# facebookresearch/multipathnet

Hardware: NVIDIA H100
Metric: proposals/sec (higher is better)
Workload: dtype fp32 (wgmma split emulation, fp32 accumulate: 3 bf16 products per MAC, 2 fp16 products in fc6/fc7)

## Files before the change

### multipathnet_b200/csrc/gemm_tc.cu

```cuda
#include "conv_gemm.cuh"
#include "wgmma.cuh"
#include "fp8_e4m3.cuh"
#include <algorithm>
#include <stdlib.h>
#include <string.h>

namespace {

constexpr int BM = 128;
constexpr int BK = 64;
constexpr int TC_THREADS = 384;
constexpr int CONS_THREADS = 256;
constexpr int A_TILE_BYTES = BM * BK * 2;
constexpr int SMEM_BUDGET = 196608;

__host__ __device__ constexpr int a_planes(OperandScheme ops) { return (ops == OperandScheme::BF16X1 || ops == OperandScheme::FP8X1) ? 1 : 2; }
__host__ __device__ constexpr int b_planes(OperandScheme ops) { return ops == OperandScheme::BF16X3 ? 2 : 1; }
__host__ __device__ constexpr int elem_bytes(OperandScheme ops) { return ops == OperandScheme::FP8X1 ? 1 : 2; }
__host__ __device__ constexpr int row_bytes(int BN, OperandScheme ops) { return (ops == OperandScheme::FP8X1 || BN == 256) ? 64 : 128; }
__host__ __device__ constexpr int stage_k(int BN, OperandScheme ops) { return row_bytes(BN, ops) / elem_bytes(ops); }
__host__ __device__ constexpr int kb_steps(int BN, OperandScheme ops) { return BK / stage_k(BN, ops); }
__host__ __device__ constexpr int a_tile_bytes(int BN, OperandScheme ops) { return BM * row_bytes(BN, ops); }
__host__ __device__ constexpr int stage_bytes(int BN, OperandScheme ops = OperandScheme::BF16X3) {
  return (a_planes(ops) * BM + b_planes(ops) * BN) * row_bytes(BN, ops);
}
__host__ __device__ constexpr int max_stages(int BN, OperandScheme ops) { return row_bytes(BN, ops) == 64 ? 8 : 4; }
__host__ __device__ constexpr int num_stages(int BN, OperandScheme ops = OperandScheme::BF16X3) {
  return (SMEM_BUDGET / stage_bytes(BN, ops)) > max_stages(BN, ops) ? max_stages(BN, ops) : (SMEM_BUDGET / stage_bytes(BN, ops));
}
constexpr int EPI_WARP_BYTES = 16 * 128;
constexpr int EPI_BYTES = (CONS_THREADS / 32) * EPI_WARP_BYTES;
__host__ __device__ constexpr int tc_smem_bytes(int BN, OperandScheme ops) {
  return num_stages(BN, ops) * stage_bytes(BN, ops) + EPI_BYTES + 1024  + 256 ;
}

struct TcParams {
  int N, Ho, Wo, Cout;
  int kh, kw, stride, pad;
  int cblocks;
  int tn, th, tw;
  int tiles_img, tiles_h, tiles_w, tiles_n;
  int units;
  const float *bias;
  const __nv_bfloat16 *res_hi, *res_lo; long long res_ld;
  __nv_bfloat16 *out_hi, *out_lo; long long out_ld;
  float *out_f32; long long out_f32_ld;
  __nv_bfloat16 *pool_hi, *pool_lo; long long pool_ld; int Hp, Wp;
  int relu;
  int splitk, kb_per_split;
  long long split_stride;
  unsigned long long *tl_min, *tl_max;
  float acc_scale;
  int out_fmt;
  unsigned *ovf;
  const int *a_exp, *b_exp; long long sample_pix;
};

__device__ __forceinline__ unsigned long long gtimer() {
  unsigned long long t; asm volatile("mov.u64 %0, %%globaltimer;" : "=l"(t)); return t;
}
__device__ __forceinline__ void tl_min_stamp(const unsigned long long *base_, int i) {
  if (base_) atomicMin(const_cast<unsigned long long *>(base_) + i, gtimer());
}
__device__ __forceinline__ void tl_max_stamp(const unsigned long long *base_, int i) {
  if (base_) atomicMax(const_cast<unsigned long long *>(base_) + i, gtimer());
}
__device__ __forceinline__ uint32_t smem_u32(const void *p) { return (uint32_t)__cvta_generic_to_shared(p); }
__device__ __forceinline__ void mbar_init(uint32_t bar, uint32_t count) {
  asm volatile("mbarrier.init.shared::cta.b64 [%0], %1;" ::"r"(bar), "r"(count) : "memory");
}
__device__ __forceinline__ void mbar_expect_tx(uint32_t bar, uint32_t bytes) {
  asm volatile("mbarrier.arrive.expect_tx.shared::cta.b64 _, [%0], %1;" ::"r"(bar), "r"(bytes) : "memory");
}
__device__ __forceinline__ void mbar_arrive(uint32_t bar) {
  asm volatile("mbarrier.arrive.shared::cta.b64 _, [%0];" ::"r"(bar) : "memory");
}
__device__ __forceinline__ void mbar_wait(uint32_t bar, uint32_t parity) {
  uint32_t done;
  uint32_t spins = 0;
  do {
    asm volatile(
        "{\n\t.reg .pred p;\n\t"
        "mbarrier.try_wait.parity.shared::cta.b64 p, [%1], %2;\n\t"
        "selp.u32 %0, 1, 0, p;\n\t}"
        : "=r"(done) : "r"(bar), "r"(parity) : "memory");
    if (!done && ++spins == (1u << 26)) __trap();
  } while (!done);
}
__device__ __forceinline__ void tma_load_4d(uint32_t dst, const CUtensorMap *tm, uint32_t bar, int c0, int c1,
                                            int c2, int c3) {
  asm volatile(
      "cp.async.bulk.tensor.4d.shared::cluster.global.mbarrier::complete_tx::bytes [%0], [%1, {%3, %4, %5, %6}], [%2];"
      ::"r"(dst), "l"(reinterpret_cast<uint64_t>(tm)), "r"(bar), "r"(c0), "r"(c1), "r"(c2), "r"(c3) : "memory");
}
__device__ __forceinline__ void tma_load_2d(uint32_t dst, const CUtensorMap *tm, uint32_t bar, int c0, int c1) {
  asm volatile(
      "cp.async.bulk.tensor.2d.shared::cluster.global.mbarrier::complete_tx::bytes [%0], [%1, {%3, %4}], [%2];"
      ::"r"(dst), "l"(reinterpret_cast<uint64_t>(tm)), "r"(bar), "r"(c0), "r"(c1) : "memory");
}
__device__ __forceinline__ void prefetch_tmap(const CUtensorMap *tm) {
  asm volatile("prefetch.tensormap [%0];" ::"l"(reinterpret_cast<uint64_t>(tm)) : "memory");
}

__device__ __forceinline__ uint64_t make_smem_desc(uint32_t saddr) {
  uint64_t d = 0;
  d |= (uint64_t)((saddr & 0x3FFFFu) >> 4);
  d |= (uint64_t)1 << 16;
  d |= (uint64_t)(1024 >> 4) << 32;
  d |= (uint64_t)1 << 62;
  return d;
}

__device__ __forceinline__ uint64_t make_smem_desc_64b(uint32_t saddr) {
  uint64_t d = 0;
  d |= (uint64_t)((saddr & 0x3FFFFu) >> 4);
  d |= (uint64_t)1 << 16;
  d |= (uint64_t)(512 >> 4) << 32;
  d |= (uint64_t)2 << 62;
  return d;
}

template <int BN, OperandScheme OPS>
__device__ __forceinline__ void mma_kstep(float (&acc)[BN / 2], uint64_t a_hi, uint64_t a_lo, uint64_t b_hi, uint64_t b_lo, bool first) {
  constexpr bool F16 = (OPS == OperandScheme::FP16X2);
#pragma unroll
  for (int k = 0; k < stage_k(BN, OPS) / 16; ++k) {
    const uint64_t adv = (uint64_t)((k * 16 * 2) >> 4);
    const uint32_t later = (first && k == 0) ? 0u : 1u;
    if constexpr (OPS == OperandScheme::BF16X1) {
      wgmma_nk16<BN, false>(acc, a_hi + adv, b_hi + adv, later);
    } else {
      wgmma_nk16<BN, F16>(acc, a_lo + adv, b_hi + adv, later);
      if (!F16) wgmma_nk16<BN, F16>(acc, a_hi + adv, b_lo + adv, 1u);
      wgmma_nk16<BN, F16>(acc, a_hi + adv, b_hi + adv, 1u);
    }
  }
}

struct UnitPos { int nt, twi, thi, tni, split; };
__device__ __forceinline__ UnitPos unit_pos(const TcParams &p, int unit) {
  UnitPos u;
  const int tile = unit / p.splitk;
  u.split = unit - tile * p.splitk;
  u.nt = tile % p.tiles_n;
  const int mt = tile / p.tiles_n;
  u.twi = mt % p.tiles_w; u.thi = (mt / p.tiles_w) % p.tiles_h; u.tni = mt / (p.tiles_w * p.tiles_h);
  return u;
}
__device__ __forceinline__ long long row_pixel(const TcParams &p, const UnitPos &u, int row, bool &ok, int *whn = nullptr) {
  const int lw = __ffs(p.tw) - 1, lh = __ffs(p.th) - 1;
  const int wl = row & (p.tw - 1), hl = (row >> lw) & (p.th - 1), nl = row >> (lw + lh);
  const int wo = u.twi * p.tw + wl, ho = u.thi * p.th + hl, n = u.tni * p.tn + nl;
  ok = (wo < p.Wo) && (ho < p.Ho) && (n < p.N);
  if (whn) { whn[0] = wo; whn[1] = ho; whn[2] = n; }
  return ((long long)n * p.Ho + ho) * p.Wo + wo;
}

__device__ __forceinline__ void store_plane_chunk(uint32_t so, const uint32_t (&v)[16], __nv_bfloat16 *out, long long ld,
                                                  const TcParams &p, const UnitPos &u, int rbase, int col0, int lane) {
  const int r = lane >> 2;
  const uint32_t wr = so + (uint32_t)(r * 128 + 4 * (lane & 3));
  __syncwarp();
#pragma unroll
  for (int j = 0; j < 8; ++j) {
    const uint32_t a = wr + (uint32_t)((j ^ r) * 16);
    asm volatile("st.shared.b32 [%0], %1;" ::"r"(a), "r"(v[j]) : "memory");
    asm volatile("st.shared.b32 [%0], %1;" ::"r"(a + 8 * 128), "r"(v[8 + j]) : "memory");
  }
  __syncwarp();
  const int row0 = lane >> 3, ch = lane & 7;
  const uint32_t rd0 = so + (uint32_t)(row0 * 128 + ((ch ^ row0) * 16)), rd1 = so + (uint32_t)(row0 * 128 + ((ch ^ row0 ^ 4) * 16));
  const bool col_ok = col0 + 8 * ch < p.Cout;
#pragma unroll
  for (int q = 0; q < 4; ++q) {
    uint4 d;
    asm volatile("ld.shared.v4.b32 {%0, %1, %2, %3}, [%4];" : "=r"(d.x), "=r"(d.y), "=r"(d.z), "=r"(d.w)
                 : "r"(((q & 1) ? rd1 : rd0) + (uint32_t)(q * 4 * 128)) : "memory");
    bool ok;
    const long long pix = row_pixel(p, u, rbase + 4 * q + row0, ok);
    if (ok && col_ok) *reinterpret_cast<uint4 *>(out + pix * ld + col0 + 8 * ch) = d;
  }
}

template <int BN, OperandScheme OPS>
__device__ __forceinline__ void tile_epilogue(const TcParams &p, const UnitPos &u, float (&acc)[BN / 2], int g, int wq,
                                              int lane, uint32_t so) {
  const int rbase = 64 * g + 16 * wq;
  const int c0 = 2 * (lane & 3);
  bool fok[2]; long long fpix[2];
#pragma unroll
  for (int i = 0; i < 2; ++i) fpix[i] = row_pixel(p, u, rbase + (lane >> 2) + 8 * i, fok[i]);
  int ea[2] = {0, 0};
  if constexpr (OPS == OperandScheme::FP8X1) {
#pragma unroll
    for (int i = 0; i < 2; ++i) ea[i] = fok[i] ? __ldg(p.a_exp + fpix[i] / p.sample_pix) : 0;
  }
  const bool pool = (p.pool_hi != nullptr);
  bool pok = false; long long ppix = 0;
  if (pool) {
    int whn[3];
    row_pixel(p, u, rbase + 2 * (lane >> 3), pok, whn);
    ppix = ((long long)whn[2] * p.Hp + (whn[1] >> 1)) * p.Wp + (whn[0] >> 1);
  }
  float *const out_f32 = p.out_f32 ? p.out_f32 + (long long)u.split * p.split_stride : nullptr;
#pragma unroll 1
  for (int m = 0; m < BN / 64; ++m) {
    const int col0 = u.nt * BN + 64 * m;
    if (col0 >= p.Cout) break;
    float *f = acc;
#pragma unroll
    for (int j = 0; j < 8; ++j) {
      const int c = col0 + 8 * j + c0;
      const bool full8 = col0 + 8 * j + 8 <= p.Cout;
      float b[2] = {0.f, 0.f};
      int eb[2] = {0, 0};
#pragma unroll
      for (int k = 0; k < 2; ++k) {
        if (p.bias && c + k < p.Cout) b[k] = __ldg(p.bias + c + k);
        if constexpr (OPS == OperandScheme::FP8X1) eb[k] = __ldg(p.b_exp + c + k);
      }
#pragma unroll
      for (int i = 0; i < 2; ++i) {
        float &f0 = f[4 * j + 2 * i], &f1 = f[4 * j + 2 * i + 1];
        if constexpr (OPS == OperandScheme::FP16X2) { f0 *= p.acc_scale; f1 *= p.acc_scale; }
        if constexpr (OPS == OperandScheme::FP8X1) {
          f0 *= mpn_fp8::pow2(-(ea[i] + eb[0])); f1 *= mpn_fp8::pow2(-(ea[i] + eb[1]));
        }
        if (p.bias) {
          if (c < p.Cout) f0 += b[0];
          if (c + 1 < p.Cout) f1 += b[1];
        }
        if (p.res_hi && full8 && fok[i]) {
          const float2 x = bf16x2_to_float2(*reinterpret_cast<const uint32_t *>(p.res_hi + fpix[i] * p.res_ld + c));
          const float2 y = bf16x2_to_float2(*reinterpret_cast<const uint32_t *>(p.res_lo + fpix[i] * p.res_ld + c));
          f0 += x.x + y.x; f1 += x.y + y.y;
        }
        if (p.relu) { f0 = fmaxf(f0, 0.f); f1 = fmaxf(f1, 0.f); }
        if (out_f32 && fok[i]) {
          float *o = out_f32 + fpix[i] * p.out_f32_ld + c;
          if (c < p.Cout) o[0] = f0;
          if (c + 1 < p.Cout) o[1] = f1;
        }
      }
    }
    float mx[16];
    if (pool) {
#pragma unroll
      for (int j = 0; j < 8; ++j)
#pragma unroll
        for (int k = 0; k < 2; ++k) {
          float top = fok[0] ? f[4 * j + k] : -INFINITY, bot = fok[1] ? f[4 * j + 2 + k] : -INFINITY;
          top = fmaxf(top, __shfl_xor_sync(0xffffffffu, top, 4));
          bot = fmaxf(bot, __shfl_xor_sync(0xffffffffu, bot, 4));
          mx[2 * j + k] = fmaxf(top, bot);
        }
    }
#pragma unroll 1
    for (int plane = 0; plane < 2; ++plane) {
      if (p.out_hi) {
        uint32_t v[16];
#pragma unroll
        for (int j = 0; j < 8; ++j)
#pragma unroll
          for (int i = 0; i < 2; ++i) {
            uint32_t hi2 = 0, lo2 = 0;
            if (fok[i]) split_x2(p.out_fmt, f[4 * j + 2 * i], f[4 * j + 2 * i + 1], hi2, lo2, p.ovf);
            v[8 * i + j] = plane ? lo2 : hi2;
          }
        store_plane_chunk(so, v, plane ? p.out_lo : p.out_hi, p.out_ld, p, u, rbase, col0, lane);
      }
      if (pool) {
        const int pr = lane >> 3;
        __syncwarp();
        if (!(lane & 4) && fok[0]) {
#pragma unroll
          for (int j = 0; j < 8; ++j) {
            uint32_t hi2, lo2;
            split_x2(p.out_fmt, mx[2 * j], mx[2 * j + 1], hi2, lo2, p.ovf);
            const uint32_t a = so + (uint32_t)(pr * 128 + ((j ^ pr) * 16) + 4 * (lane & 3));
            asm volatile("st.shared.b32 [%0], %1;" ::"r"(a), "r"(plane ? lo2 : hi2) : "memory");
          }
        }
        __syncwarp();
        const int ch = lane & 7;
        uint4 d;
        asm volatile("ld.shared.v4.b32 {%0, %1, %2, %3}, [%4];" : "=r"(d.x), "=r"(d.y), "=r"(d.z), "=r"(d.w)
                     : "r"(so + (uint32_t)(pr * 128 + ((ch ^ pr) * 16))) : "memory");
        if (pok && col0 + 8 * ch < p.Cout)
          *reinterpret_cast<uint4 *>((plane ? p.pool_lo : p.pool_hi) + ppix * p.pool_ld + col0 + 8 * ch) = d;
      }
    }
#pragma unroll
    for (int k = 0; k + 32 < BN / 2; ++k) acc[k] = acc[k + 32];
  }
}

template <int BN, OperandScheme OPS = OperandScheme::BF16X3>
__global__ void __launch_bounds__(TC_THREADS, 1)
conv_gemm_tc_kernel(const __grid_constant__ CUtensorMap tmA_hi, const __grid_constant__ CUtensorMap tmA_lo,
                    const __grid_constant__ CUtensorMap tmB_hi, const __grid_constant__ CUtensorMap tmB_lo,
                    const TcParams p) {
  constexpr int S = num_stages(BN, OPS);
  constexpr int STAGE = stage_bytes(BN, OPS);
  constexpr int A_TILE = a_tile_bytes(BN, OPS);
  constexpr int B_TILE_BYTES = BN * row_bytes(BN, OPS);
  constexpr int B_OFF = a_planes(OPS) * A_TILE;
  constexpr int KSTEPS = kb_steps(BN, OPS);
  static_assert(S >= 2 && 2 * S * 8 <= 256, "ring depth: at least two stages, barriers in their 256 bytes");
  extern __shared__ uint8_t smem_raw[];
  uint8_t *smem = reinterpret_cast<uint8_t *>((reinterpret_cast<uintptr_t>(smem_raw) + 1023) & ~(uintptr_t)1023);
  uint64_t *bars = reinterpret_cast<uint64_t *>(smem + (size_t)S * STAGE + EPI_BYTES);
  const uint32_t smem_base = smem_u32(smem);
  const uint32_t bar_base = smem_u32(bars);
  auto full_bar = [&](int s) { return bar_base + 8u * s; };
  auto empty_bar = [&](int s) { return bar_base + 8u * (S + s); };

  const int tid = threadIdx.x, lane = tid & 31;
  const int num_kb = p.kh * p.kw * p.cblocks;

  if (tid == 0) {
    tl_min_stamp(p.tl_min, 0);
    if (a_planes(OPS) == 1) { prefetch_tmap(&tmA_hi); prefetch_tmap(&tmB_hi); }
    else { prefetch_tmap(&tmA_hi); prefetch_tmap(&tmA_lo); prefetch_tmap(&tmB_hi); prefetch_tmap(&tmB_lo); }
    for (int s = 0; s < S; ++s) { mbar_init(full_bar(s), 1); mbar_init(empty_bar(s), CONS_THREADS / 32); }
    asm volatile("fence.mbarrier_init.release.cluster;" ::: "memory");
  }
  __syncthreads();
  asm volatile("griddepcontrol.wait;" ::: "memory");
  asm volatile("griddepcontrol.launch_dependents;" ::: "memory");
  if (tid == 0) tl_min_stamp(p.tl_min, 1);

  if (tid < 128) {
    asm volatile("setmaxnreg.dec.sync.aligned.u32 24;" ::: "memory");
    if (tid == 0) {
      int it = 0;
      for (int unit = (int)blockIdx.x; unit < p.units; unit += (int)gridDim.x) {
        const UnitPos u = unit_pos(p, unit);
        const int kb0 = u.split * p.kb_per_split, kb1 = min(num_kb, kb0 + p.kb_per_split);
        const int w_in0 = u.twi * p.tw * p.stride - p.pad, h_in0 = u.thi * p.th * p.stride - p.pad, n0 = u.tni * p.tn;
        const int b_row0 = u.nt * BN;
        for (int kb = kb0; kb < kb1; ++kb) {
          const int tap = kb / p.cblocks, cb = kb - tap * p.cblocks;
          const int khi = tap / p.kw, kwi = tap - khi * p.kw;
#pragma unroll
          for (int h = 0; h < KSTEPS; ++h, ++it) {
            const int s = it % S; const uint32_t ph = (uint32_t)(it / S) & 1u;
            const int ka = cb * BK + h * stage_k(BN, OPS), kk = kb * BK + h * stage_k(BN, OPS);
            mbar_wait(empty_bar(s), ph ^ 1u);
            const uint32_t sa = smem_base + (uint32_t)s * STAGE;
            mbar_expect_tx(full_bar(s), (uint32_t)STAGE);
            tma_load_4d(sa, &tmA_hi, full_bar(s), ka, w_in0 + kwi, h_in0 + khi, n0);
            if (a_planes(OPS) == 2) tma_load_4d(sa + A_TILE, &tmA_lo, full_bar(s), ka, w_in0 + kwi, h_in0 + khi, n0);
            tma_load_2d(sa + B_OFF, &tmB_hi, full_bar(s), kk, b_row0);
            if (b_planes(OPS) == 2) tma_load_2d(sa + B_OFF + B_TILE_BYTES, &tmB_lo, full_bar(s), kk, b_row0);
          }
        }
      }
    }
    return;
  }

  asm volatile("setmaxnreg.inc.sync.aligned.u32 240;" ::: "memory");
  const int e = tid - 128;
  const int g = e >> 7, wq = (e >> 5) & 3;
  const uint32_t so = smem_base + (uint32_t)(S * STAGE + (e >> 5) * EPI_WARP_BYTES);
  int it = 0;
  for (int unit = (int)blockIdx.x; unit < p.units; unit += (int)gridDim.x) {
    const UnitPos u = unit_pos(p, unit);
    const int kb0 = u.split * p.kb_per_split, kb1 = min(num_kb, kb0 + p.kb_per_split);
    float acc[BN / 2];
#pragma unroll
    for (int i = 0; i < BN / 2; ++i) acc[i] = 0.f;
    if constexpr (OPS == OperandScheme::FP8X1) {
      float part[BN / 2];
#pragma unroll
      for (int i = 0; i < BN / 2; ++i) part[i] = 0.f;
      for (int kb = kb0; kb < kb1; ++kb, ++it) {
        const int s = it % S; const uint32_t ph = (uint32_t)(it / S) & 1u;
        mbar_wait(full_bar(s), ph);
        if (it == 0 && e == 0) tl_min_stamp(p.tl_min, 2);
        const uint32_t sa = smem_base + (uint32_t)s * STAGE;
        const uint64_t a8 = make_smem_desc_64b(sa + (uint32_t)g * (A_TILE / 2));
        const uint64_t b8 = make_smem_desc_64b(sa + B_OFF);
#pragma unroll
        for (int k = 0; k < BK / 32; ++k) {
          wgmma_fence_acc(part);
          wgmma_fence();
          wgmma_e4m3_nk32<BN>(part, a8 + (uint64_t)(2 * k), b8 + (uint64_t)(2 * k), 0u);
          wgmma_commit();
          wgmma_wait<0>();
          wgmma_fence_acc(part);
#pragma unroll
          for (int i = 0; i < BN / 2; ++i) acc[i] += part[i];
        }
        if (lane == 0) mbar_arrive(empty_bar(s));
      }
    } else {
      const int steps = (kb1 - kb0) * KSTEPS;
      for (int i = 0; i < steps; ++i, ++it) {
        const int s = it % S; const uint32_t ph = (uint32_t)(it / S) & 1u;
        mbar_wait(full_bar(s), ph);
        if (it == 0 && e == 0) tl_min_stamp(p.tl_min, 2);
        const uint32_t sa = smem_base + (uint32_t)s * STAGE;
        auto desc = [](uint32_t a) { return row_bytes(BN, OPS) == 64 ? make_smem_desc_64b(a) : make_smem_desc(a); };
        const uint64_t a_hi = desc(sa + (uint32_t)g * (A_TILE / 2));
        const uint64_t a_lo = desc(sa + A_TILE + (uint32_t)g * (A_TILE / 2));
        const uint64_t b_hi = desc(sa + B_OFF);
        const uint64_t b_lo = desc(sa + B_OFF + B_TILE_BYTES);
        wgmma_fence_acc(acc);
        wgmma_fence();
        mma_kstep<BN, OPS>(acc, a_hi, a_lo, b_hi, b_lo, i == 0);
        wgmma_commit();
        wgmma_wait<1>();
        wgmma_fence_acc(acc);
        if (i > 0 && lane == 0) mbar_arrive(empty_bar((it - 1) % S));
      }
      wgmma_wait<0>();
      wgmma_fence_acc(acc);
      if (lane == 0) mbar_arrive(empty_bar((it - 1) % S));
    }
    if (e == 0) tl_max_stamp(p.tl_max, 0);
    const uint32_t t_epi = (p.tl_max && e == 0) ? (uint32_t)gtimer() : 0u;
    tile_epilogue<BN, OPS>(p, u, acc, g, wq, lane, so);
    if (e == 0) {
      tl_max_stamp(p.tl_max, 1);
      if (p.tl_max) atomicAdd(p.tl_max + 3, (unsigned long long)((uint32_t)gtimer() - t_epi));
    }
  }
}


constexpr int C1_THREADS = 256;
constexpr int C1_A_BYTES = 2 * A_TILE_BYTES;
constexpr int C1_B_BYTES = 2 * 64 * 128;
constexpr int C1_OUT_WARP = 16 * 128;
constexpr int C1_SMEM = 2 * C1_A_BYTES + C1_B_BYTES + (C1_THREADS / 32) * C1_OUT_WARP + 1024;

__device__ __forceinline__ void conv1_gather(const float *__restrict__ x, int pix, int pixels, int H, int W, int bhalf,
                                             float (&in)[16]) {
#pragma unroll
  for (int k = 0; k < 16; ++k) in[k] = 0.f;
  if (pix < pixels) {
    const int HW = H * W;
    const int n = pix / HW, rem = pix - n * HW;
    const int ho = rem / W, wo = rem - ho * W;
    const float *x0 = x + ((size_t)n * 3 * HW + (size_t)(ho - 1) * W + (wo - 1));
    const bool rok[3] = {ho >= 1, true, ho + 1 < H}, cok[3] = {wo >= 1, true, wo + 1 < W};
#pragma unroll
    for (int k = 0; k < 16; ++k) {
      const int kk = 16 * bhalf + k;
      if (kk < 27) {
        const int ci = kk / 9, r = (kk / 3) % 3, q = kk % 3;
        in[k] = (rok[r] && cok[q]) ? __ldg(x0 + ci * HW + r * W + q) : 0.f;
      }
    }
  }
}

__device__ __forceinline__ void conv1_store_plane(uint32_t so, const uint32_t (&v)[16], __nv_bfloat16 *out, int pix0,
                                                  int pixels, int lane) {
  const int r = lane >> 2;
  const uint32_t wr = so + (uint32_t)(r * 128 + 4 * (lane & 3));
  __syncwarp();
#pragma unroll
  for (int j = 0; j < 8; ++j) {
    const uint32_t a = wr + (uint32_t)((j ^ r) * 16);
    asm volatile("st.shared.b32 [%0], %1;" ::"r"(a), "r"(v[j]) : "memory");
    asm volatile("st.shared.b32 [%0], %1;" ::"r"(a + 8 * 128), "r"(v[8 + j]) : "memory");
  }
  __syncwarp();
  const int row0 = lane >> 3, ch = lane & 7;
  const uint32_t rd0 = so + (uint32_t)(row0 * 128 + ((ch ^ row0) * 16)), rd1 = so + (uint32_t)(row0 * 128 + ((ch ^ row0 ^ 4) * 16));
  __nv_bfloat16 *o = out + (size_t)(pix0 + row0) * 64 + ch * 8;
#pragma unroll
  for (int q = 0; q < 4; ++q) {
    uint4 d;
    asm volatile("ld.shared.v4.b32 {%0, %1, %2, %3}, [%4];" : "=r"(d.x), "=r"(d.y), "=r"(d.z), "=r"(d.w)
                 : "r"(((q & 1) ? rd1 : rd0) + (uint32_t)(q * 4 * 128)) : "memory");
    if (pix0 + row0 + 4 * q < pixels) *reinterpret_cast<uint4 *>(o + q * 4 * 64) = d;
  }
}

__global__ void __launch_bounds__(C1_THREADS, 2)
conv1_tc_kernel(const float *__restrict__ x, int N, int H, int W, const float *__restrict__ w, const float *__restrict__ bias,
                int relu, __nv_bfloat16 *__restrict__ out_hi, __nv_bfloat16 *__restrict__ out_lo) {
  extern __shared__ uint8_t smem_raw[];
  uint8_t *smem = reinterpret_cast<uint8_t *>((reinterpret_cast<uintptr_t>(smem_raw) + 1023) & ~(uintptr_t)1023);
  uint8_t *sB = smem + 2 * C1_A_BYTES;
  const int tid = threadIdx.x, lane = tid & 31, warp = tid >> 5;
  const uint32_t so = smem_u32(sB + C1_B_BYTES) + (uint32_t)(warp * C1_OUT_WARP);
  const uint32_t b_base = smem_u32(sB);
  const int g = tid >> 7;
  const int pixels = N * H * W;
  const int total_tiles = (pixels + BM - 1) / BM;
  asm volatile("griddepcontrol.wait;" ::: "memory");
  asm volatile("griddepcontrol.launch_dependents;" ::: "memory");
  const int c0 = 2 * (lane & 3);
  for (int i = tid; i < 64 * 4; i += C1_THREADS) {
    const int row = i >> 2, j = i & 3;
    uint32_t hh[4], ll[4];
#pragma unroll
    for (int q = 0; q < 4; ++q) {
      const int k0 = j * 8 + 2 * q;
      const float v0 = (k0 < 27) ? __ldg(w + row * 27 + k0) : 0.f, v1 = (k0 + 1 < 27) ? __ldg(w + row * 27 + k0 + 1) : 0.f;
      split_bf16x2(v0, v1, hh[q], ll[q]);
    }
    const uint32_t off = (uint32_t)row * 128u + (uint32_t)((j ^ (row & 7)) * 16);
    *reinterpret_cast<uint4 *>(sB + off) = make_uint4(hh[0], hh[1], hh[2], hh[3]);
    *reinterpret_cast<uint4 *>(sB + 64 * 128 + off) = make_uint4(ll[0], ll[1], ll[2], ll[3]);
  }
  const int brow = tid & 127, bhalf = tid >> 7;
  float in[16];
  conv1_gather(x, (int)blockIdx.x * BM + brow, pixels, H, W, bhalf, in);
  for (int tile = blockIdx.x, it = 0; tile < total_tiles; tile += gridDim.x, ++it) {
    uint8_t *sa = smem + (it & 1) * C1_A_BYTES;
    uint8_t *pa = sa + (size_t)brow * 128;
#pragma unroll
    for (int jj = 0; jj < 2; ++jj) {
      const int j = 2 * bhalf + jj;
      uint32_t hh[4], ll[4];
#pragma unroll
      for (int q = 0; q < 4; ++q) split_bf16x2(in[jj * 8 + 2 * q], in[jj * 8 + 2 * q + 1], hh[q], ll[q]);
      const int pj = (j ^ (brow & 7)) * 16;
      *reinterpret_cast<uint4 *>(pa + pj) = make_uint4(hh[0], hh[1], hh[2], hh[3]);
      *reinterpret_cast<uint4 *>(pa + A_TILE_BYTES + pj) = make_uint4(ll[0], ll[1], ll[2], ll[3]);
    }
    asm volatile("fence.proxy.async.shared::cta;" ::: "memory");
    __syncthreads();
    float acc[32];
#pragma unroll
    for (int i = 0; i < 32; ++i) acc[i] = 0.f;
    const uint32_t a_base = smem_u32(sa);
    const uint64_t a_hi = make_smem_desc(a_base + (uint32_t)g * (A_TILE_BYTES / 2));
    const uint64_t a_lo = make_smem_desc(a_base + A_TILE_BYTES + (uint32_t)g * (A_TILE_BYTES / 2));
    const uint64_t b_hi = make_smem_desc(b_base), b_lo = make_smem_desc(b_base + 64 * 128);
    wgmma_fence_acc(acc);
    wgmma_fence();
#pragma unroll
    for (int k = 0; k < 2; ++k) {
      const uint64_t adv = (uint64_t)((k * 16 * 2) >> 4);
      wgmma_nk16<64, false>(acc, a_lo + adv, b_hi + adv, k ? 1u : 0u);
      wgmma_nk16<64, false>(acc, a_hi + adv, b_lo + adv, 1u);
      wgmma_nk16<64, false>(acc, a_hi + adv, b_hi + adv, 1u);
    }
    wgmma_commit();
    const int next = tile + (int)gridDim.x;
    conv1_gather(x, next < total_tiles ? next * BM + brow : pixels, pixels, H, W, bhalf, in);
    wgmma_wait<0>();
    wgmma_fence_acc(acc);
#pragma unroll
    for (int j = 0; j < 8; ++j) {
      const float2 b = __ldg(reinterpret_cast<const float2 *>(bias + 8 * j + c0));
#pragma unroll
      for (int h = 0; h < 2; ++h) {
        float &f0 = acc[4 * j + 2 * h], &f1 = acc[4 * j + 2 * h + 1];
        f0 += b.x; f1 += b.y;
        if (relu) { f0 = fmaxf(f0, 0.f); f1 = fmaxf(f1, 0.f); }
      }
    }
    const int pix0 = tile * BM + 64 * g + 16 * (warp & 3);
#pragma unroll 1
    for (int plane = 0; plane < 2; ++plane) {
      uint32_t v[16];
#pragma unroll
      for (int j = 0; j < 8; ++j)
#pragma unroll
        for (int h = 0; h < 2; ++h) {
          uint32_t hi2, lo2;
          split_bf16x2(acc[4 * j + 2 * h], acc[4 * j + 2 * h + 1], hi2, lo2);
          v[8 * h + j] = plane ? lo2 : hi2;
        }
      conv1_store_plane(so, v, plane ? out_lo : out_hi, pix0, pixels, lane);
    }
  }
}

struct ReduceParams {
  const float *ws; long long split_stride; int splitk; long long pixels; int Cout;
  const float *bias; const __nv_bfloat16 *res_hi, *res_lo; long long res_ld; int relu;
  __nv_bfloat16 *out_hi, *out_lo; long long out_ld; float *out_f32; long long out_f32_ld;
  OutScatter scatter;
};
__global__ void __launch_bounds__(256) splitk_reduce_kernel(const ReduceParams r) {
  MPN_PDL_SYNC();
  const long long idx = (long long)blockIdx.x * blockDim.x + threadIdx.x;
  if (idx >= r.pixels * r.Cout) return;
  const long long pix = idx / r.Cout; const int c = (int)(idx - pix * r.Cout);
  float acc = 0.f;
  for (int s = 0; s < r.splitk; ++s) acc += r.ws[(long long)s * r.split_stride + idx];
  if (r.bias) acc += __ldg(r.bias + c);
  if (r.res_hi) acc += join_bf16(r.res_hi[pix * r.res_ld + c], r.res_lo[pix * r.res_ld + c]);
  if (r.relu) acc = fmaxf(acc, 0.f);
  if (r.out_hi) { __nv_bfloat16 h, l; split_bf16(acc, h, l); r.out_hi[pix * r.out_ld + c] = h; r.out_lo[pix * r.out_ld + c] = l; }
  if (r.scatter.n > 0) {
#pragma unroll 1
    for (int g = 0; g < r.scatter.n; ++g)
      if (c >= r.scatter.seg[g].c0 && c < r.scatter.seg[g].c1) { r.scatter.seg[g].ptr[pix * r.scatter.seg[g].ld + (c - r.scatter.seg[g].c0)] = acc; break; }
  } else if (r.out_f32) r.out_f32[pix * r.out_f32_ld + c] = acc;
}

typedef CUresult (*PFN_encodeTiled)(CUtensorMap *, CUtensorMapDataType, cuuint32_t, void *, const cuuint64_t *,
                                    const cuuint64_t *, const cuuint32_t *, const cuuint32_t *, CUtensorMapInterleave,
                                    CUtensorMapSwizzle, CUtensorMapL2promotion, CUtensorMapFloatOOBfill);
PFN_encodeTiled get_encode_fn() {
  static PFN_encodeTiled fn = nullptr;
  if (!fn) {
    void *p = nullptr; cudaDriverEntryPointQueryResult q;
    if (cudaGetDriverEntryPoint("cuTensorMapEncodeTiled", &p, cudaEnableDefault, &q) == cudaSuccess &&
        q == cudaDriverEntryPointSuccess)
      fn = reinterpret_cast<PFN_encodeTiled>(p);
  }
  return fn;
}

int encode_map(mpn_ctx *ctx, CUtensorMap *tm, const void *base, int rank, const cuuint64_t *dims,
               const cuuint64_t *strides_bytes , const cuuint32_t *box, const cuuint32_t *estr, int BN, OperandScheme ops) {
  const bool fp8 = ops == OperandScheme::FP8X1;
  PFN_encodeTiled fn = get_encode_fn();
  if (!fn) return mpn_fail(ctx, MPN_ERR_CUDA, "cuTensorMapEncodeTiled entry point unavailable");
  CUresult r = fn(tm, fp8 ? CU_TENSOR_MAP_DATA_TYPE_UINT8 : CU_TENSOR_MAP_DATA_TYPE_BFLOAT16, (cuuint32_t)rank, const_cast<void *>(base), dims,
                  strides_bytes, box, estr, CU_TENSOR_MAP_INTERLEAVE_NONE, row_bytes(BN, ops) == 64 ? CU_TENSOR_MAP_SWIZZLE_64B : CU_TENSOR_MAP_SWIZZLE_128B,
                  CU_TENSOR_MAP_L2_PROMOTION_L2_256B, CU_TENSOR_MAP_FLOAT_OOB_FILL_NONE);
  if (r != CUDA_SUCCESS) {
    char b[256];
    snprintf(b, sizeof b, "cuTensorMapEncodeTiled failed (%d): rank %d dims %llu %llu box %u %u", (int)r, rank,
             (unsigned long long)dims[0], (unsigned long long)dims[1], box[0], box[1]);
    return mpn_fail(ctx, MPN_ERR_CUDA, b);
  }
  return MPN_OK;
}

inline bool tc_use_pdl() {
  static const int on = [] { const char *e = getenv("MPN_TC_PDL"); return (e && e[0] == '0') ? 0 : 1; }();
  return on != 0;
}

template <int BN, OperandScheme OPS = OperandScheme::BF16X3>
int launch_bn(mpn_ctx *ctx, const ConvPlan &pl, const TcParams &tp) {
  const int smem = tc_smem_bytes(BN, OPS);
  constexpr int bslot = BN == 256 ? 2 : (BN == 128 ? 1 : 0);
  constexpr int slot = OPS == OperandScheme::FP16X2 ? 3 : (OPS == OperandScheme::BF16X1 ? 5 + bslot
                                                         : (OPS == OperandScheme::FP8X1 ? 8 + bslot : bslot));
  if (!ctx->tc_attr_set[slot]) {
    MPN_CUDA(ctx, cudaFuncSetAttribute(conv_gemm_tc_kernel<BN, OPS>, cudaFuncAttributeMaxDynamicSharedMemorySize, smem));
    ctx->tc_attr_set[slot] = 1;
  }
  const long long units = (long long)pl.tiles_img * pl.tiles_h * pl.tiles_w * pl.tiles_n * pl.splitk;
  MPN_CHECK_ARG(ctx, units > 0 && units < (1ll << 31), "conv_tc: grid size out of range");
  TcParams tpu = tp;
  tpu.units = (int)units;
  cudaLaunchConfig_t cfg = {};
  cfg.gridDim = dim3((unsigned)std::min<long long>(units, ctx->sm_count));
  cfg.blockDim = dim3(TC_THREADS); cfg.dynamicSmemBytes = (size_t)smem; cfg.stream = ctx->stream;
  cudaLaunchAttribute attr[1];
  int na = 0;
  if (tc_use_pdl()) {
    attr[na].id = cudaLaunchAttributeProgrammaticStreamSerialization;
    attr[na].val.programmaticStreamSerializationAllowed = 1;
    ++na;
  }
  cfg.attrs = attr; cfg.numAttrs = na;
  MPN_CUDA(ctx, cudaLaunchKernelEx(&cfg, conv_gemm_tc_kernel<BN, OPS>, pl.tmA_hi, pl.tmA_lo, pl.tmB_hi, pl.tmB_lo, tpu));
  MPN_LAUNCHED(ctx);
  return MPN_OK;
}

int launch_ops(mpn_ctx *ctx, const ConvPlan &pl, const TcParams &tp) {
  if (pl.ops == OperandScheme::FP16X2) return launch_bn<256, OperandScheme::FP16X2>(ctx, pl, tp);
  if (pl.ops == OperandScheme::FP8X1)
    return pl.BN == 128 ? launch_bn<128, OperandScheme::FP8X1>(ctx, pl, tp) : launch_bn<64, OperandScheme::FP8X1>(ctx, pl, tp);
  if (pl.ops == OperandScheme::BF16X1) {
    switch (pl.BN) {
      case 256: return launch_bn<256, OperandScheme::BF16X1>(ctx, pl, tp);
      case 128: return launch_bn<128, OperandScheme::BF16X1>(ctx, pl, tp);
      default: return launch_bn<64, OperandScheme::BF16X1>(ctx, pl, tp);
    }
  }
  switch (pl.BN) {
    case 256: return launch_bn<256>(ctx, pl, tp);
    case 128: return launch_bn<128>(ctx, pl, tp);
    default: return launch_bn<64>(ctx, pl, tp);
  }
}

}

int conv1_tc_launch(mpn_ctx *ctx, const float *x_nchw, int N, int H, int W, const float *w_dev, const float *bias_dev, int relu,
                    DTensor &y) {
  MPN_CHECK_ARG(ctx, y.hi && y.lo && y.C == 64 && y.ld % 8 == 0, "conv1_tc: output must be 64-channel split planes");
  MPN_CHECK_ARG(ctx, bias_dev, "conv1_tc: bias missing");
  MPN_CHECK_ARG(ctx, y.ld == 64 && (long long)N * H * W < (1ll << 31) - 256, "conv1_tc: dense 64-channel output and < 2^31 pixels");
  if (!ctx->tc_attr_set[4]) {
    MPN_CUDA(ctx, cudaFuncSetAttribute(conv1_tc_kernel, cudaFuncAttributeMaxDynamicSharedMemorySize, C1_SMEM));
    ctx->tc_attr_set[4] = 1;
  }
  const long long tiles = ((long long)N * H * W + BM - 1) / BM;
  cudaLaunchConfig_t cfg = {};
  cfg.gridDim = dim3((unsigned)std::min<long long>(tiles, 2ll * ctx->sm_count)); cfg.blockDim = dim3(C1_THREADS);
  cfg.dynamicSmemBytes = (size_t)C1_SMEM; cfg.stream = ctx->stream;
  cudaLaunchAttribute attr[1];
  int na = 0;
  if (tc_use_pdl()) { attr[na].id = cudaLaunchAttributeProgrammaticStreamSerialization; attr[na].val.programmaticStreamSerializationAllowed = 1; ++na; }
  cfg.attrs = attr; cfg.numAttrs = na;
  MPN_CUDA(ctx, cudaLaunchKernelEx(&cfg, conv1_tc_kernel, x_nchw, N, H, W, w_dev, bias_dev, relu, y.hi, y.lo));
  MPN_LAUNCHED(ctx);
  return MPN_OK;
}

double conv_flops(const ConvProblem &p) {
  const double Ho = (double)p.y.H, Wo = (double)p.y.W;
  return 2.0 * (double)p.x.C * p.Cout * p.kh * p.kw * Ho * Wo * (double)p.y.N;
}

static int conv_tc_plan_impl(mpn_ctx *ctx, int sm_count, const ConvProblem &p, ConvPlan &pl, bool choose_only) {
  pl.valid = 0;
  MPN_CHECK_ARG(ctx, choose_only || (p.x.hi && p.x.lo && ((p.w_hi && p.w_lo) || p.w16)), "conv_tc: operands must be split-bf16 (or an fp16 weight plane)");
  MPN_CHECK_ARG(ctx, !(p.w16 && p.bf16), "conv_tc: the bf16 numerics do not take an fp16 weight plane");
  MPN_CHECK_ARG(ctx, !(p.fp8 && (p.w16 || p.bf16)), "conv_tc: the fp8 numerics take neither an fp16 weight plane nor the bf16 numerics");
  MPN_CHECK_ARG(ctx, choose_only || !p.fp8 || (p.x8 && p.x8_exp && p.w8 && p.w8_exp), "conv_tc: the fp8 numerics need e4m3 planes and exponents");
  pl.ops = p.w16 ? OperandScheme::FP16X2 : (p.fp8 ? OperandScheme::FP8X1 : (p.bf16 ? OperandScheme::BF16X1 : OperandScheme::BF16X3));
  const bool w16 = pl.ops == OperandScheme::FP16X2, fp8 = pl.ops == OperandScheme::FP8X1;
  MPN_CHECK_ARG(ctx, choose_only || (p.x.fmt == 1) == w16, "conv_tc: fp16 activation planes go with the fp16 weight plane (and only with it)");
  MPN_CHECK_ARG(ctx, p.x.C % BK == 0, "conv_tc: Cin must be a multiple of 64");
  MPN_CHECK_ARG(ctx, p.x.ld % 8 == 0, "conv_tc: input pixel stride must be a multiple of 8 elements");
  MPN_CHECK_ARG(ctx, p.stride >= 1 && p.stride <= 2, "conv_tc: stride must be 1 or 2");
  const int Ho = (int)p.y.H, Wo = (int)p.y.W, N = (int)p.y.N;
  pl.flat = (p.kh == 1 && p.kw == 1 && p.stride == 1 && p.pad == 0) ? 1 : 0;
  pl.mode = 0; pl.splitk = 1;
  cuuint64_t dims[4], strides[3]; cuuint32_t box[4], estr[4];
  int gtn = 1, gth = 1, gtw = BM;
  if (!pl.flat) {
    double best = -1.0;
    for (int tw = 1; tw <= 128; tw <<= 1)
      for (int th = 1; th * tw <= 128; th <<= 1) {
        const int tn = 128 / (tw * th);
        if (tw * p.stride > 256 || th * p.stride > 256) continue;
        const long long tiles = (long long)((Wo + tw - 1) / tw) * ((Ho + th - 1) / th) * ((N + tn - 1) / tn);
        const double util = (double)N * Ho * Wo / (double)(tiles * 128) + 1e-6 * tw;
        if (util > best) { best = util; gtn = tn; gth = th; gtw = tw; }
      }
  }
  const long long P = (long long)p.x.N * p.x.H * p.x.W;
  {
    const bool r3_ok = (p.kh == 3 && p.kw == 3 && p.stride == 1 && p.pad == 1);
    const char *env3 = getenv("MPN_TC_R3");
    const char *env3m = getenv("MPN_TC_R3_MINPIX");
    const long long r3_minpix = env3m ? atoll(env3m) : 0;
    pl.mode = (r3_ok && !(env3 && env3[0] == '0') && P >= r3_minpix) ? 1 : 0;
  }
  const long long tiles_m = pl.flat ? (P + BM - 1) / BM
                                    : (pl.mode ? (long long)((Wo + 7) / 8) * ((Ho + 15) / 16) * N
                                               : (long long)((Wo + gtw - 1) / gtw) * ((Ho + gth - 1) / gth) * ((N + gtn - 1) / gtn));
  {
    const int taps = p.kh * p.kw;
    const double kblocks = (double)taps * (double)(p.x.C / BK);
    double best = 1e300; int best_bn = 64;
    for (int bi = 0; bi < 3; ++bi) {
      const int bn = bi == 0 ? 256 : (bi == 1 ? 128 : 64);
      if (w16 && bn != 256) continue;
      if (fp8 && bn == 256) continue;
      if (!p.m_invariant && bn > 64 && bn > ((p.Cout + 63) / 64) * 64) continue;
      const int roi_bn = p.Cout > 128 ? 256 : (p.Cout > 64 ? 128 : 64);
      if (p.m_invariant && bn != (fp8 ? std::min(roi_bn, 128) : roi_bn)) continue;
      const long long units = tiles_m * ((p.Cout + bn - 1) / bn);
      const long long rounds = (units + sm_count - 1) / sm_count;
      const double mma = (w16 ? 2.0 : (pl.ops == OperandScheme::BF16X1 ? 1.0 : (fp8 ? 0.5 : 3.0))) * 128.0 * bn * 64.0 / 1024.0;
      const double ingest = ((double)a_planes(pl.ops) * 128 + (double)b_planes(pl.ops) * bn) * (fp8 ? 64.0 : 128.0) / 48.0;
      const double cost = (double)rounds * (kblocks * std::max(mma, ingest) + 1500.0 + 8.0 * bn);
      if (cost < best * 0.999) { best = cost; best_bn = bn; }
    }
    pl.BN = best_bn;
    pl.tiles_n = (p.Cout + pl.BN - 1) / pl.BN;
  }
  if (pl.flat) {
    pl.tn = 1; pl.th = 1; pl.tw = BM;
    pl.tiles_img = 1; pl.tiles_h = 1; pl.tiles_w = (int)((P + BM - 1) / BM);
    dims[0] = (cuuint64_t)p.x.C; dims[1] = (cuuint64_t)P; dims[2] = 1; dims[3] = 1;
    strides[0] = (cuuint64_t)p.x.ld * 2; strides[1] = (cuuint64_t)P * p.x.ld * 2; strides[2] = strides[1];
    box[0] = (cuuint32_t)stage_k(pl.BN, pl.ops); box[1] = BM; box[2] = 1; box[3] = 1;
    estr[0] = estr[1] = estr[2] = estr[3] = 1;
  } else {
    if (pl.mode == 1) { pl.tn = 1; pl.th = 16; pl.tw = 8; }
    else { pl.tn = gtn; pl.th = gth; pl.tw = gtw; }
    pl.tiles_w = (Wo + pl.tw - 1) / pl.tw; pl.tiles_h = (Ho + pl.th - 1) / pl.th; pl.tiles_img = (N + pl.tn - 1) / pl.tn;
    dims[0] = (cuuint64_t)p.x.C; dims[1] = (cuuint64_t)p.x.W; dims[2] = (cuuint64_t)p.x.H; dims[3] = (cuuint64_t)p.x.N;
    strides[0] = (cuuint64_t)p.x.ld * 2; strides[1] = (cuuint64_t)p.x.W * p.x.ld * 2;
    strides[2] = (cuuint64_t)p.x.H * p.x.W * p.x.ld * 2;
    box[0] = (cuuint32_t)stage_k(pl.BN, pl.ops); box[1] = (cuuint32_t)(pl.tw * p.stride); box[2] = (cuuint32_t)(pl.th * p.stride); box[3] = (cuuint32_t)pl.tn;
    estr[0] = 1; estr[1] = (cuuint32_t)p.stride; estr[2] = (cuuint32_t)p.stride; estr[3] = 1;
  }
  {
    const long long units = tiles_m * pl.tiles_n;
    const long long num_kb = (long long)p.kh * p.kw * (p.x.C / BK);
    long long sk = std::min<long long>(num_kb / 8, 8);
    if (p.m_invariant) { if (!(pl.flat && p.Cout <= 128) || sk < 2) sk = 1; }
    else if (p.wide_k_split && pl.flat && num_kb >= 256)
      sk = std::max<long long>({1, std::min<long long>(sm_count / units, num_kb / 8), (num_kb + 31) / 32});
    else if (pl.mode == 1 || sk < 2 || units * sk > sm_count) sk = 1;
    const char *env2 = getenv("MPN_TC_SPLITK");
    if (env2 && env2[0] == '0') sk = 1;
    pl.splitk = (int)std::max<long long>(sk, 1);
    pl.kb_per_split = (int)((num_kb + pl.splitk - 1) / pl.splitk);
    pl.splitk = (int)((num_kb + pl.kb_per_split - 1) / pl.kb_per_split);
  }
  if (choose_only) return MPN_OK;
  const long long Ktot = (long long)p.kh * p.kw * p.x.C;
  cuuint64_t bd[2] = {(cuuint64_t)Ktot, (cuuint64_t)p.Cout}, bs[1] = {(cuuint64_t)Ktot * 2};
  cuuint32_t bb[2] = {(cuuint32_t)stage_k(pl.BN, pl.ops), (cuuint32_t)pl.BN}, be[2] = {1, 1};
  if (fp8) {
    const cuuint64_t C8 = (cuuint64_t)p.x.C;
    if (pl.flat) { strides[0] = C8; strides[1] = (cuuint64_t)P * C8; strides[2] = strides[1]; }
    else { strides[0] = C8; strides[1] = (cuuint64_t)p.x.W * C8; strides[2] = (cuuint64_t)p.x.H * p.x.W * C8; }
    bs[0] = (cuuint64_t)Ktot;
    MPN_TRY(encode_map(ctx, &pl.tmA_hi, p.x8, 4, dims, strides, box, estr, pl.BN, pl.ops));
    MPN_TRY(encode_map(ctx, &pl.tmB_hi, p.w8, 2, bd, bs, bb, be, pl.BN, pl.ops));
// ... 92 lines not shown
```

Before: 414,100.

## Add ping-pong consumer warpgroup schedule for persistent conv GEMM tiles

Adds a ping-pong variant of the TC conv kernel. Each of the two consumer warpgroups now owns alternate whole tiles and computes both 64-row halves (two accumulator sets), instead of both warpgroups splitting every tile. Named barriers order the warpgroups so one runs its epilogue while the other issues wgmma, hiding epilogue latency. It is used only for 16-bit schemes with BN<=128 when there are at least two units per CTA. It doubles accumulator register pressure (up to 128 floats) and adds barrier coordination, which risks spills or serialization.

```diff
diff --git a/multipathnet_b200/csrc/gemm_tc.cu b/multipathnet_b200/csrc/gemm_tc.cu
--- a/multipathnet_b200/csrc/gemm_tc.cu
+++ b/multipathnet_b200/csrc/gemm_tc.cu
@@ -120,22 +120,32 @@
   return d;
 }
 
-template <int BN, OperandScheme OPS>
-__device__ __forceinline__ void mma_kstep(float (&acc)[BN / 2], uint64_t a_hi, uint64_t a_lo, uint64_t b_hi, uint64_t b_lo, bool first) {
+template <int BN, OperandScheme OPS, int NH>
+__device__ __forceinline__ void mma_kstep(float (&acc)[NH][BN / 2], const uint64_t (&a_hi)[NH], const uint64_t (&a_lo)[NH],
+                                          uint64_t b_hi, uint64_t b_lo, bool first) {
   constexpr bool F16 = (OPS == OperandScheme::FP16X2);
 #pragma unroll
   for (int k = 0; k < stage_k(BN, OPS) / 16; ++k) {
     const uint64_t adv = (uint64_t)((k * 16 * 2) >> 4);
     const uint32_t later = (first && k == 0) ? 0u : 1u;
     if constexpr (OPS == OperandScheme::BF16X1) {
-      wgmma_nk16<BN, false>(acc, a_hi + adv, b_hi + adv, later);
+#pragma unroll
+      for (int h = 0; h < NH; ++h) wgmma_nk16<BN, false>(acc[h], a_hi[h] + adv, b_hi + adv, later);
     } else {
-      wgmma_nk16<BN, F16>(acc, a_lo + adv, b_hi + adv, later);
-      if (!F16) wgmma_nk16<BN, F16>(acc, a_hi + adv, b_lo + adv, 1u);
-      wgmma_nk16<BN, F16>(acc, a_hi + adv, b_hi + adv, 1u);
-    }
-  }
-}
+#pragma unroll
+      for (int h = 0; h < NH; ++h) wgmma_nk16<BN, F16>(acc[h], a_lo[h] + adv, b_hi + adv, later);
+      if (!F16) {
+#pragma unroll
+        for (int h = 0; h < NH; ++h) wgmma_nk16<BN, F16>(acc[h], a_hi[h] + adv, b_lo + adv, 1u);
+      }
+#pragma unroll
+      for (int h = 0; h < NH; ++h) wgmma_nk16<BN, F16>(acc[h], a_hi[h] + adv, b_hi + adv, 1u);
+    }
+  }
+}
+
+__device__ __forceinline__ void named_bar_sync(int id) { asm volatile("bar.sync %0, 256;" ::"r"(id) : "memory"); }
+__device__ __forceinline__ void named_bar_arrive(int id) { asm volatile("bar.arrive %0, 256;" ::"r"(id) : "memory"); }
 
 struct UnitPos { int nt, twi, thi, tni, split; };
 __device__ __forceinline__ UnitPos unit_pos(const TcParams &p, int unit) {
@@ -295,11 +305,14 @@
   }
 }
 
-template <int BN, OperandScheme OPS = OperandScheme::BF16X3>
+template <int BN, OperandScheme OPS = OperandScheme::BF16X3, bool PP = false>
 __global__ void __launch_bounds__(TC_THREADS, 1)
 conv_gemm_tc_kernel(const __grid_constant__ CUtensorMap tmA_hi, const __grid_constant__ CUtensorMap tmA_lo,
                     const __grid_constant__ CUtensorMap tmB_hi, const __grid_constant__ CUtensorMap tmB_lo,
                     const TcParams p) {
+  static_assert(!PP || (BN <= 128 && (OPS == OperandScheme::BF16X3 || OPS == OperandScheme::BF16X1)),
+                "ping-pong: 16-bit schemes with at most 128 accumulators per thread");
+  constexpr int NH = PP ? 2 : 1;
   constexpr int S = num_stages(BN, OPS);
   constexpr int STAGE = stage_bytes(BN, OPS);
   constexpr int A_TILE = a_tile_bytes(BN, OPS);
@@ -322,7 +335,7 @@
     tl_min_stamp(p.tl_min, 0);
     if (a_planes(OPS) == 1) { prefetch_tmap(&tmA_hi); prefetch_tmap(&tmB_hi); }
     else { prefetch_tmap(&tmA_hi); prefetch_tmap(&tmA_lo); prefetch_tmap(&tmB_hi); prefetch_tmap(&tmB_lo); }
-    for (int s = 0; s < S; ++s) { mbar_init(full_bar(s), 1); mbar_init(empty_bar(s), CONS_THREADS / 32); }
+    for (int s = 0; s < S; ++s) { mbar_init(full_bar(s), 1); mbar_init(empty_bar(s), CONS_THREADS / 32 / NH); }
     asm volatile("fence.mbarrier_init.release.cluster;" ::: "memory");
   }
   __syncthreads();
@@ -363,14 +376,21 @@
   asm volatile("setmaxnreg.inc.sync.aligned.u32 240;" ::: "memory");
   const int e = tid - 128;
   const int g = e >> 7, wq = (e >> 5) & 3;
+  const bool wg_lead = (e & 127) == 0;
   const uint32_t so = smem_base + (uint32_t)(S * STAGE + (e >> 5) * EPI_WARP_BYTES);
   int it = 0;
-  for (int unit = (int)blockIdx.x; unit < p.units; unit += (int)gridDim.x) {
+  int j = 0;
+  for (int unit = (int)blockIdx.x; unit < p.units; unit += (int)gridDim.x, ++j) {
     const UnitPos u = unit_pos(p, unit);
     const int kb0 = u.split * p.kb_per_split, kb1 = min(num_kb, kb0 + p.kb_per_split);
-    float acc[BN / 2];
-#pragma unroll
-    for (int i = 0; i < BN / 2; ++i) acc[i] = 0.f;
+    if (PP && (j & 1) != g) { it += (kb1 - kb0) * KSTEPS; continue; }
+    if (PP && j > 0) named_bar_sync(1 + g);
+    const bool first_unit = PP ? j == g : unit == (int)blockIdx.x;
+    float acc[NH][BN / 2];
+#pragma unroll
+    for (int h = 0; h < NH; ++h)
+#pragma unroll
+      for (int i = 0; i < BN / 2; ++i) acc[h][i] = 0.f;
     if constexpr (OPS == OperandScheme::FP8X1) {
       float part[BN / 2];
 #pragma unroll
@@ -378,7 +398,7 @@
       for (int kb = kb0; kb < kb1; ++kb, ++it) {
         const int s = it % S; const uint32_t ph = (uint32_t)(it / S) & 1u;
         mbar_wait(full_bar(s), ph);
-        if (it == 0 && e == 0) tl_min_stamp(p.tl_min, 2);
+        if (first_unit && kb == kb0 && wg_lead) tl_min_stamp(p.tl_min, 2);
         const uint32_t sa = smem_base + (uint32_t)s * STAGE;
         const uint64_t a8 = make_smem_desc_64b(sa + (uint32_t)g * (A_TILE / 2));
         const uint64_t b8 = make_smem_desc_64b(sa + B_OFF);
@@ -391,7 +411,7 @@
           wgmma_wait<0>();
           wgmma_fence_acc(part);
 #pragma unroll
-          for (int i = 0; i < BN / 2; ++i) acc[i] += part[i];
+          for (int i = 0; i < BN / 2; ++i) acc[0][i] += part[i];
         }
         if (lane == 0) mbar_arrive(empty_bar(s));
       }
@@ -400,31 +420,45 @@
       for (int i = 0; i < steps; ++i, ++it) {
         const int s = it % S; const uint32_t ph = (uint32_t)(it / S) & 1u;
         mbar_wait(full_bar(s), ph);
-        if (it == 0 && e == 0) tl_min_stamp(p.tl_min, 2);
+        if (first_unit && i == 0 && wg_lead) tl_min_stamp(p.tl_min, 2);
         const uint32_t sa = smem_base + (uint32_t)s * STAGE;
         auto desc = [](uint32_t a) { return row_bytes(BN, OPS) == 64 ? make_smem_desc_64b(a) : make_smem_desc(a); };
-        const uint64_t a_hi = desc(sa + (uint32_t)g * (A_TILE / 2));
-        const uint64_t a_lo = desc(sa + A_TILE + (uint32_t)g * (A_TILE / 2));
+        uint64_t a_hi[NH], a_lo[NH];
+#pragma unroll
+        for (int h = 0; h < NH; ++h) {
+          const uint32_t half = (uint32_t)(PP ? h : g) * (A_TILE / 2);
+          a_hi[h] = desc(sa + half);
+          a_lo[h] = desc(sa + A_TILE + half);
+        }
         const uint64_t b_hi = desc(sa + B_OFF);
         const uint64_t b_lo = desc(sa + B_OFF + B_TILE_BYTES);
-        wgmma_fence_acc(acc);
+#pragma unroll
+        for (int h = 0; h < NH; ++h) wgmma_fence_acc(acc[h]);
         wgmma_fence();
-        mma_kstep<BN, OPS>(acc, a_hi, a_lo, b_hi, b_lo, i == 0);
+        mma_kstep<BN, OPS, NH>(acc, a_hi, a_lo, b_hi, b_lo, i == 0);
         wgmma_commit();
         wgmma_wait<1>();
-        wgmma_fence_acc(acc);
+#pragma unroll
+        for (int h = 0; h < NH; ++h) wgmma_fence_acc(acc[h]);
         if (i > 0 && lane == 0) mbar_arrive(empty_bar((it - 1) % S));
       }
+      if (PP && unit + (int)gridDim.x < p.units) named_bar_arrive(2 - g);
       wgmma_wait<0>();
-      wgmma_fence_acc(acc);
+#pragma unroll
+      for (int h = 0; h < NH; ++h) wgmma_fence_acc(acc[h]);
       if (lane == 0) mbar_arrive(empty_bar((it - 1) % S));
     }
-    if (e == 0) tl_max_stamp(p.tl_max, 0);
-    const uint32_t t_epi = (p.tl_max && e == 0) ? (uint32_t)gtimer() : 0u;
-    tile_epilogue<BN, OPS>(p, u, acc, g, wq, lane, so);
-    if (e == 0) {
+    if (wg_lead) tl_max_stamp(p.tl_max, 0);
+    const uint32_t t_epi = (p.tl_max && wg_lead) ? (uint32_t)gtimer() : 0u;
+#pragma unroll 1
+    for (int h = 0; h < NH; ++h) {
+      tile_epilogue<BN, OPS>(p, u, acc[0], PP ? h : g, wq, lane, so);
+#pragma unroll
+      for (int i = 0; i < BN / 2; ++i) acc[0][i] = acc[NH - 1][i];
+    }
+    if (wg_lead) {
       tl_max_stamp(p.tl_max, 1);
-      if (p.tl_max) atomicAdd(p.tl_max + 3, (unsigned long long)((uint32_t)gtimer() - t_epi));
+      if (p.tl_max && (PP || g == 0)) atomicAdd(p.tl_max + 3, (unsigned long long)((uint32_t)gtimer() - t_epi));
     }
   }
 }
@@ -638,19 +672,26 @@
 template <int BN, OperandScheme OPS = OperandScheme::BF16X3>
 int launch_bn(mpn_ctx *ctx, const ConvPlan &pl, const TcParams &tp) {
   const int smem = tc_smem_bytes(BN, OPS);
+  const long long units = (long long)pl.tiles_img * pl.tiles_h * pl.tiles_w * pl.tiles_n * pl.splitk;
+  MPN_CHECK_ARG(ctx, units > 0 && units < (1ll << 31), "conv_tc: grid size out of range");
+  const long long grid = std::min<long long>(units, ctx->sm_count);
+  constexpr bool pp_ok = BN <= 128 && (OPS == OperandScheme::BF16X3 || OPS == OperandScheme::BF16X1);
+  const bool pp = pp_ok && units >= 2 * grid;
   constexpr int bslot = BN == 256 ? 2 : (BN == 128 ? 1 : 0);
   constexpr int slot = OPS == OperandScheme::FP16X2 ? 3 : (OPS == OperandScheme::BF16X1 ? 5 + bslot
                                                          : (OPS == OperandScheme::FP8X1 ? 8 + bslot : bslot));
-  if (!ctx->tc_attr_set[slot]) {
-    MPN_CUDA(ctx, cudaFuncSetAttribute(conv_gemm_tc_kernel<BN, OPS>, cudaFuncAttributeMaxDynamicSharedMemorySize, smem));
-    ctx->tc_attr_set[slot] = 1;
-  }
-  const long long units = (long long)pl.tiles_img * pl.tiles_h * pl.tiles_w * pl.tiles_n * pl.splitk;
-  MPN_CHECK_ARG(ctx, units > 0 && units < (1ll << 31), "conv_tc: grid size out of range");
+  constexpr int pp_slot = (OPS == OperandScheme::BF16X1 ? 12 : 10) + bslot;
+  auto kern = conv_gemm_tc_kernel<BN, OPS, false>;
+  if constexpr (pp_ok) { if (pp) kern = conv_gemm_tc_kernel<BN, OPS, true>; }
+  const int kslot = pp ? pp_slot : slot;
+  if (!ctx->tc_attr_set[kslot]) {
+    MPN_CUDA(ctx, cudaFuncSetAttribute(kern, cudaFuncAttributeMaxDynamicSharedMemorySize, smem));
+    ctx->tc_attr_set[kslot] = 1;
+  }
   TcParams tpu = tp;
   tpu.units = (int)units;
   cudaLaunchConfig_t cfg = {};
-  cfg.gridDim = dim3((unsigned)std::min<long long>(units, ctx->sm_count));
+  cfg.gridDim = dim3((unsigned)grid);
   cfg.blockDim = dim3(TC_THREADS); cfg.dynamicSmemBytes = (size_t)smem; cfg.stream = ctx->stream;
   cudaLaunchAttribute attr[1];
   int na = 0;
@@ -660,7 +701,7 @@
     ++na;
   }
   cfg.attrs = attr; cfg.numAttrs = na;
-  MPN_CUDA(ctx, cudaLaunchKernelEx(&cfg, conv_gemm_tc_kernel<BN, OPS>, pl.tmA_hi, pl.tmA_lo, pl.tmB_hi, pl.tmB_lo, tpu));
+  MPN_CUDA(ctx, cudaLaunchKernelEx(&cfg, kern, pl.tmA_hi, pl.tmA_lo, pl.tmB_hi, pl.tmB_lo, tpu));
   MPN_LAUNCHED(ctx);
   return MPN_OK;
 }
```

Result: faster. 419,900, median of 6 (+1.4%).
